# vedrocks15/Gradient-Based-Path-Tracing

Hardware: AMD Instinct MI355X
Metric: GDPT Msamples/s (base+4 offset) + Poisson ms, cbox 512x512 (higher is better)
Workload: dtype f64

## Files before the change

gradient-based-path-tracing_amd/csrc/hip/capi_device.hip:

```cpp
#include "../../../include/gdpt.h"
#include "../capi_common.h"
#include "../device_scene.h"
#include "../host/scene_prepare.h"
#include "poisson_kernels.h"
#include "recon_l1.h"
#include "recon_weighted.h"
#include "render_kernels.h"
#include "scene_internal.h"

#include <hip/hip_runtime.h>

#include <algorithm>
#include <cmath>
#include <cstdlib>
#include <cstring>
#include <exception>
#include <memory>
#include <string>
#include <thread>
#include <vector>

namespace {

using gdpt::ck;
// ... 178 lines not shown
            if (!capturing) join_scratch(sc);
            sc->need_fence = true;
        }
        ss.partials.alloc(need, "hipMalloc(work-item partials)");
    }
    if (!overlap) {
        if (!capturing) {
            sc->join();
            if (ss.used) ck(hipStreamWaitEvent(stream, ss.released, 0), "hipStreamWaitEvent(launch scratch)");
        }
    } else {
        if (sc->have_caller && stream != sc->last_caller) {
            for (auto &o : sc->scratch) ck(hipStreamWaitEvent(stream, o.rendered, 0), "hipStreamWaitEvent(render stream)");
            sc->need_fence = true;
        }
        if (sc->need_fence || !prev_entry) {
            for (auto &st : sc->render_stream) ck(hipStreamWaitEvent(st, entry, 0), "hipStreamWaitEvent(fence)");
            sc->need_fence = false;
        } else
            ck(hipStreamWaitEvent(sc->render_stream[k], prev_entry, 0), "hipStreamWaitEvent(previous call)");
        if (ss.used) ck(hipStreamWaitEvent(sc->render_stream[k], ss.released, 0), "hipStreamWaitEvent(launch scratch)");
    }
    sc->have_caller = true; sc->last_caller = stream;
    return ss;
}

gdpt::RenderLaunch begin_launch(GdptScene *sc, const Band &b, bool path, int take_pct, hipStream_t stream, const GdptRenderStats *stats, ScratchClaim *claim) {
    auto knob = [](const char *name, int def) { return gdpt::debug_knob_int(name, def); };
    const DevSceneView &v = sc->view;
    gdpt::RouteInputs in{};
    in.path = path; in.rng_scheme = b.rng; in.shift_mode = b.shift; in.max_depth = b.max_depth; in.rr_depth = v.rr_depth;
    in.one_sided = sc->traits.one_sided; in.has_rough = sc->traits.has_rough; in.lambert_only = sc->traits.lambert_only; in.material_mask = sc->traits.material_mask;
    in.has_spheres = v.num_spheres != 0; in.const_textures = v.all_textures_constant != 0; in.has_envmap = v.has_envmap != 0;
    in.fits_lds = gdpt::scene_fits_lds(v.num_nodes, v.num_prims, v.num_tris, v.num_materials, v.num_lights, sc->traits.bvh_depth);
    in.fits_lds_wide = gdpt::scene_fits_lds_wide(v.num_nodes4, v.num_prims, v.num_tris, v.num_materials, v.num_lights, sc->traits.wide_stack_need);
    in.force_eager = knob("force_eager", 0) != 0; in.no_lds_scene = knob("no_lds_scene", 0) != 0; in.lds_wide = knob("lds_wide", 1) != 0;
// ... 6 lines not shown
    rl.spp = b.spp; rl.stream_spp = b.stream_spp; rl.first_sample = b.first_sample; rl.row_begin = b.row_begin; rl.row_end = b.row_end; rl.max_depth = b.max_depth;
    rl.count_traversal = stats && stats->nodes_visited == ~0ull;
    rl.force_log2k = knob("log2k", -1);
    rl.thresh_a = knob("keep_frac", -1); rl.thresh_c = knob("search_frac", -1);
    rl.num_cus = sc->num_cus; rl.blocks_per_cu = knob("blocks_per_cu", 0);
    const bool capturing = is_capturing(stream);
    const bool overlap = !stats && gdpt::can_overlap(rl.route) && !capturing && knob("no_render_overlap", 0) == 0;
    size_t need = 0;
    if (gdpt::is_persistent(rl.route)) {
        rl.plan = gdpt::make_chunk_plan(b.spp, rl.force_log2k, (long long)v.cam.width * b.plan_rows, gdpt::resident_lanes(rl), take_pct);
        need = (size_t)16 * (size_t)gdpt::band_slots(v.cam.width, b.row_end - b.row_begin) * (size_t)rl.plan.n;
    }
    GdptLaunchScratch &ss = claim_scratch(sc, overlap, capturing, need, stream);
    rl.counters = ss.counters; sc->d_counters = ss.counters;
    if (gdpt::is_persistent(rl.route)) { rl.partials = ss.partials; rl.queue_head = ss.queue; }
    if (overlap) { rl.kernel_stream = sc->render_stream[sc->overlapped & 1]; rl.kernel_done = ss.rendered; }
    claim->set = &ss; claim->record_release = !capturing;
    return rl;
}

void run_launch(GdptScene *sc, const gdpt::RenderLaunch &rl, const ScratchClaim &claim, const Band &b, hipStream_t stream, GdptRenderStats *stats) {
    const bool stamped = gdpt::is_stamped(rl.route);
    const hipStream_t ks = rl.kernel_stream ? rl.kernel_stream : stream;
    if (rl.kernel_stream) sc->in_flight = true;
    ck(hipMemsetAsync(rl.counters, 0, sizeof(gdpt::RenderCounters), ks), "hipMemsetAsync(counters)");
    if (stamped) ck(hipMemsetAsync(&rl.counters->stamps[12], 0xFF, 2 * sizeof(unsigned long long), ks), "hipMemsetAsync(stamps)");
    if (stats) ck(hipEventRecord(sc->ev0, stream), "hipEventRecord");
    gdpt::launch_render(sc->view, rl, stream);
    if (rl.kernel_stream) sc->overlapped++;
    if (claim.record_release) { ck(hipEventRecord(claim.set->released, stream), "hipEventRecord(launch scratch)"); claim.set->used = true; }
    if (!stats) return;
    ck(hipEventRecord(sc->ev1, stream), "hipEventRecord");
    ck(hipMemcpyAsync(sc->h_counters, rl.counters, sizeof(gdpt::RenderCounters), hipMemcpyDeviceToHost, stream), "hipMemcpyAsync(counters)");
    ck(hipStreamSynchronize(stream), "hipStreamSynchronize(render)");
    float ms = 0;
    ck(hipEventElapsedTime(&ms, sc->ev0, sc->ev1), "hipEventElapsedTime");
    const gdpt::RenderCounters &c = *sc->h_counters;
    std::memset(stats, 0, sizeof(*stats));
    stats->samples = (uint64_t)sc->view.cam.width * (uint64_t)(b.row_end - b.row_begin) * (uint64_t)b.spp;
    stats->rays = c.rays; stats->bounces = c.bounces; stats->nonfinite_samples = c.nonfinite;
// ... 449 lines not shown
```

gradient-based-path-tracing_amd/csrc/hip/device_trace.h:

```cpp
#pragma once
#include "device_bsdf.h"

namespace gd {

struct Hit { float t, u, v, ngx, ngy, ngz; int gid; };

struct TraceCounters { unsigned nodes, prims, node_trips, leaf_trips, wave_steps, lane_steps; };
GD bool wave_leader() { return (int)(threadIdx.x & 63) == __ffsll((unsigned long long)__ballot(1)) - 1; }

GD bool tri_hit(const float o[3], const float d[3], float tnear, float tfar, const DevPrim &tr, float &t, float &u, float &v) {
#pragma clang fp contract(off)
    const float *e1 = tr.e1, *e2 = tr.e2;
    float px = d[1] * e2[2] - d[2] * e2[1];
    float py = d[2] * e2[0] - d[0] * e2[2];
    float pz = d[0] * e2[1] - d[1] * e2[0];
    float det = e1[0] * px + e1[1] * py + e1[2] * pz;
    if (!(det != 0.0f)) return false;
    float inv = 1.0f / det;
    float sx = o[0] - tr.v0[0], sy = o[1] - tr.v0[1], sz = o[2] - tr.v0[2];
    u = (sx * px + sy * py + sz * pz) * inv;
    if (!(u >= 0.0f && u <= 1.0f)) return false;
    float qx = sy * e1[2] - sz * e1[1];
    float qy = sz * e1[0] - sx * e1[2];
    float qz = sx * e1[1] - sy * e1[0];
// ... 170 lines not shown
GD D2 filter_sample(int type, double param, double rx, double ry) {
    D2 o;
    if (type == GDPT_FILTER_BOX) { o.x = (2 * rx - 1) * (param / 2); o.y = (2 * ry - 1) * (param / 2); }
    else if (type == GDPT_FILTER_GAUSSIAN) {
        double r = param * sqrt(-2 * log(fmax(rx, 1e-8)));
        double s, c;
        sincospi(2.0 * ry, &s, &c);
        o.x = r * c; o.y = r * s;
    } else {
        double h = param / 2;
        o.x = rx < 0.5 ? h * (sqrt(2 * rx) - 1) : h * (1 - sqrt(1 - 2 * (rx - 0.5)));
        o.y = ry < 0.5 ? h * (sqrt(2 * ry) - 1) : h * (1 - sqrt(1 - 2 * (ry - 0.5)));
    }
    return o;
}
GD D3 xform_point(const double *m, D3 p) {
    double tx = m[0] * p.x + m[1] * p.y + m[2] * p.z + m[3];
    double ty = m[4] * p.x + m[5] * p.y + m[6] * p.z + m[7];
    double tz = m[8] * p.x + m[9] * p.y + m[10] * p.z + m[11];
    double tw = m[12] * p.x + m[13] * p.y + m[14] * p.z + m[15];
    double inv_w = 1.0 / tw;
    return mk(tx * inv_w, ty * inv_w, tz * inv_w);
}
GD D3 xform_vector(const double *m, D3 v) {
    return mk(m[0] * v.x + m[1] * v.y + m[2] * v.z, m[4] * v.x + m[5] * v.y + m[6] * v.z, m[8] * v.x + m[9] * v.y + m[10] * v.z);
}
struct FilterCache { double dx, dy, ox, oy; };
template <bool PIXEL_SPACE = false>
GD Ray sample_primary(const DevCamera &cam, double sx, double sy, FilterCache *cache = nullptr, bool store = false) {
    const bool exact = PIXEL_SPACE && cam.pow2_film != 0;
    if (PIXEL_SPACE && !exact) { sx = sx / cam.width; sy = sy / cam.height; }
    double ppx = exact ? sx : sx * cam.width, ppy = exact ? sy : sy * cam.height;
    double fx = floor(ppx), fy = floor(ppy);
    D2 off;
    if (cache && !store && cache->dx == ppx - fx && cache->dy == ppy - fy) { off.x = cache->ox; off.y = cache->oy; }
    else {
        off = filter_sample(cam.filter_type, cam.filter_param, ppx - fx, ppy - fy);
        if (cache && store) { cache->dx = ppx - fx; cache->dy = ppy - fy; cache->ox = off.x; cache->oy = off.y; }
    }
    double rx, ry;
    if (exact) { rx = (fx + 0.5 + off.x) * cam.inv_width; ry = (fy + 0.5 + off.y) * cam.inv_height; }
    else { rx = (fx + 0.5 + off.x) / cam.width; ry = (fy + 0.5 + off.y) / cam.height; }
    D3 pt = xform_point(cam.sample_to_cam, mk(rx, ry, 0.0));
    D3 dir = normalize(pt);
    Ray r;
    r.org = mk(cam.org[0], cam.org[1], cam.org[2]);
    r.dir = normalize(xform_vector(cam.cam_to_world, dir));
    r.tnear = 0; r.tfar = __builtin_huge_val();
    return r;
}

}
```

gradient-based-path-tracing_amd/csrc/hip/render_device.h:

```cpp
#pragma once
#include "render_kernels.h"
#include "device_trace.h"
#include "../leaf_cursor.h"

namespace gd {

constexpr int kBlock = 256;
constexpr int kLdsSceneBytes = 20 * 1024;
constexpr int kLdsSceneLevels = 12;

struct LaneCounters { unsigned rays, bounces, nonfinite; };

enum { SEG_QUEUE = 0, SEG_TRACE = 1, SEG_VERTEX = 2, SEG_CONSUME = 3, SEG_BSDF = 4, SEG_FINISH = 5, SEG_CAMERA = 6, SEG_STEPS = 7, SEG_PUBLISH = 8, SEG_TAKE = 9, SEG_ITEM = 10, SEG_COUNT = 12, SEG_T_START = 12, SEG_T_DRY = 13, SEG_T_END = 14, SEG_SLOTS = 16 };
template <bool ON> struct Stamps {
    unsigned long long *slot;
    GD void start(unsigned long long *wave_row) {
        if (ON) { slot = wave_row; if ((threadIdx.x & 63) == 0) { for (int i = 0; i < SEG_COUNT; i++) slot[i] = 0; slot[SEG_COUNT] = __builtin_amdgcn_s_memtime(); } }
    }
    GD void mark(int seg) {
        if (ON) {
            __builtin_amdgcn_sched_barrier(0);
            const unsigned long long t = __builtin_amdgcn_s_memtime();
            __builtin_amdgcn_s_waitcnt(0xC07F);
            if ((int)(threadIdx.x & 63) == __ffsll((unsigned long long)__ballot(1)) - 1) { slot[seg] += t - slot[SEG_COUNT]; slot[SEG_COUNT] = t; }
// ... 556 lines not shown
            }
            if (!stop) {
                L.throughput = L.throughput * (G * f) / (p2 * rr_prob);
                L.num_vertices++;
                if (first) L.mats = (L.mats & 0xFFF) | ((nv.material_id & 0xFFF) << 12);
                if (!loop_allows(max_depth, L.num_vertices)) stop = true;
            }
        }
        if (!stop) act = ACT_BOUNCE;
        else if (first) { L.kc = C_AFTER_BOUNCE1 << 2; act = ACT_OFFSETS; }
        else { acc_no_offsets(acc, lp.radiance(), L.contrib, L.prob, spp, lc); act = ACT_NEXT_SAMPLE; }
    }
    stamps.mark(SEG_CONSUME);
    const bool off_valid = (st0 == S_OFFSET) && hit && nv.material_id == L.mat0();
    const bool off_resample = off_valid && (L.cmode() == C_AFTER_BOUNCE1 || L.cmode() == C_BROKE_BOUNCE2);
    bool sampled = false;
    BsdfSample bs; bs.dir_out = splat(0); bs.eta = 0; bs.roughness = 0;
    D3 f = splat(0);
    double pdf = 0;
    if (act == ACT_BOUNCE || off_resample) {
        D2 ruv; double rw;
        if (act == ACT_BOUNCE) {
            lc.bounces++;
            Pcg r; r.state = L.rng_state; r.inc = L.rng_inc;
            ruv.x = pcg_real(r); ruv.y = pcg_real(r); rw = pcg_real(r);
            L.rng_state = r.state;
            if (SERIAL_RNG && L.num_vertices == 3) { L.ruv1 = ruv; L.rw1 = rw; }
        } else if (SERIAL_RNG) { ruv = L.ruv1; rw = L.rw1; }
        else {
            Pcg r2 = pcg_init(base + (unsigned long long)L.s);
            (void)pcg_next(r2); (void)pcg_next(r2);
            ruv.x = pcg_real(r2); ruv.y = pcg_real(r2); rw = pcg_real(r2);
        }
        const D3 dir_view = -ray.dir;
// ... 15 lines not shown
            }
            if (alive) { cX = c0 * jac; wgt = L.prob / (L.prob + 1.0 * jac); }
        }
        bool flagged = (L.kc & kKcNonfinite) != 0;
        acc_offset(acc, k, L.contrib, cX, wgt, L.prob, spp, lc, flagged);
        if (flagged) L.kc |= kKcNonfinite;
        if (k == 3) { acc_base(acc, lp.radiance(), L.prob, spp, lc, flagged); L.kc &= ~kKcNonfinite; act = ACT_NEXT_SAMPLE; }
        else { L.kc = (L.kc & ~3) | (k + 1); act = ACT_OFFSET_RAY; }
    } else if (act == ACT_BOUNCE) {
        if (!sampled) act = ACT_NEXT_SAMPLE;
        else {
            if (pdf <= 0) {
                if (L.num_vertices == 3) { L.kc = C_BROKE_BOUNCE1 << 2; act = ACT_OFFSETS; }
                else if (L.num_vertices == 4 && L.mat0() == L.mat1()) { L.kc = C_BROKE_BOUNCE2 << 2; act = ACT_OFFSETS; }
                else { acc_no_offsets(acc, lp.radiance(), L.contrib, L.prob, spp, lc); act = ACT_NEXT_SAMPLE; }
            } else {
                L.org = nv.position; L.dir = bs.dir_out; L.f = f; L.pdf = pdf; L.st = S_BOUNCE;
            }
        }
    }
    stamps.mark(SEG_FINISH);
    if (act == ACT_OFFSETS) { L.kc &= ~3; act = ACT_OFFSET_RAY; }
    if (act == ACT_NEXT_SAMPLE) {
        L.s++;
        if (L.s >= L.s_end) L.st = S_DONE; else act = ACT_PRIMARY_RAY;
    }
    if (L.st == S_BOUNCE && act == ACT_BOUNCE) trav_init(sv, tv, __builtin_huge_val());
    return act;
}

template <bool SERIAL_RNG, class STAMPS = Stamps<false>>
GD void lane_camera(const DevSceneView &sv, int act, int x, int y, unsigned long long base, Lane &L, Trav &tv, LanePriv &lp, STAMPS *stp = nullptr) {
    STAMPS none{}; STAMPS &stamps = stp ? *stp : none;
    const DevCamera &cam = sv.cam;
    if (act == ACT_PRIMARY_RAY || act == ACT_OFFSET_RAY) {
        double rx, ry;
        int ox = 0, oy = 0;
        if (act == ACT_PRIMARY_RAY) {
            Pcg r;
            if (!SERIAL_RNG) r = pcg_init(base + (unsigned long long)L.s);
            else { r.state = L.rng_state; r.inc = L.rng_inc; }
            rx = pcg_real(r); ry = pcg_real(r);
            L.rng_state = r.state; L.rng_inc = r.inc;
            if (SERIAL_RNG) { L.rng_x = rx; L.rng_y = ry; }
            L.st = S_PRIMARY;
        } else {
            if (SERIAL_RNG) { rx = L.rng_x; ry = L.rng_y; }
            else { Pcg r2 = pcg_init(base + (unsigned long long)L.s); rx = pcg_real(r2); ry = pcg_real(r2); }
            const int k = L.k();
            ox = (k == 0) ? -1 : (k == 1 ? 1 : 0); oy = (k == 2) ? 1 : (k == 3 ? -1 : 0);
            L.st = S_OFFSET;
        }
        FilterCache fc;
        if (act == ACT_OFFSET_RAY) fc = lp.fc();
        Ray r = sample_primary<true>(cam, (x + ox) + rx, (y + oy) + ry, &fc, act == ACT_PRIMARY_RAY);
        if (act == ACT_PRIMARY_RAY) lp.set_fc(fc);
        L.org = r.org; L.dir = r.dir;
        trav_init(sv, tv, __builtin_huge_val());
    }
    stamps.mark(SEG_CAMERA);
}

template <bool LAMBERT, bool SERIAL_RNG, class ACC, class STAMPS = Stamps<false>, int PLAIN = 0>
GD void lane_step(const DevSceneView &sv, const TraceCtx &tx, int max_depth, double spp, int x, int y, unsigned long long base,
                  Lane &L, Trav &tv, LanePriv &lp, ACC &acc, LaneCounters &lc, TraceCounters &tc, STAMPS *stp = nullptr) {
    const int act = lane_consume<LAMBERT, SERIAL_RNG, ACC, STAMPS, PLAIN>(sv, tx, max_depth, spp, base, L, tv, lp, acc, lc, tc, stp);
    lane_camera<SERIAL_RNG, STAMPS>(sv, act, x, y, base, L, tv, lp, stp);
}

GD bool lane_tracing(int st) { return st == S_PRIMARY || st == S_BOUNCE || st == S_OFFSET; }
template <class TC>
GD void trace_pending(const DevSceneView &sv, const TraceCtx &tx, const Lane &L, Trav &tv, int keep_frac, int search_frac, TraceCounters &tc) {
    const bool pending = lane_tracing(L.st) && tv.cur != kTravDone;
    const unsigned long long m = __ballot(pending);
    if (m == 0ull) return;
    const int stop_below = (__popcll(m) * keep_frac) >> 8;
    if (pending) trav_run<TC>(sv, tx, L.org, L.dir, (L.st == S_BOUNCE) ? (float)sv.isect_eps : 0.0f, __builtin_huge_valf(), tv, stop_below, search_frac, tc);
}
GD bool lane_ready(const Lane &L, const Trav &tv) { return L.st == S_START || (lane_tracing(L.st) && tv.cur == kTravDone); }

GD unsigned wave_sum_u32(unsigned v) {
#pragma unroll
// ... 107 lines not shown
                next = (long long)got;
                end = min((long long)got + want, a.num_items);
                seen_head = end;
                if (next >= a.num_items) { exhausted = true; end = next; }
            }
            const int avail = (int)(end - next);
            const int rank = __popcll(m_idle & ((1ull << (tid & 63)) - 1ull));
            if (idle && rank < avail) item = next + rank;
            const int n_idle = __popcll(m_idle);
            next += (n_idle < avail) ? n_idle : avail;
        }
        return item;
    }
};

template <bool LAMBERT, bool LDS_SCENE, bool WIDE, bool WW, bool STAMPED = false, int PLAIN = 0, int LEAF_K = (LDS_SCENE && !GDPT_SPEC_LEAF ? GDPT_LDS_LEAF_K : 0)>
__global__ __launch_bounds__(kBlock, 2) void gdpt_render_phases(DevSceneView sv, KernelArgs a) {
    __shared__ int s_stack_fixed[LDS_SCENE ? kLdsSceneLevels * kBlock : 1];
    __shared__ __attribute__((aligned(16))) unsigned char s_scene[LDS_SCENE ? kLdsSceneBytes : 16];
    __shared__ double s_acc[15 * kBlock];
    __shared__ double s_priv[kPrivDoubles * kBlock];
    __shared__ int s_chunks[66];
    extern __shared__ __attribute__((aligned(16))) unsigned char s_dyn[];
    int *s_stack = LDS_SCENE ? s_stack_fixed : (int *)s_dyn;
    const int tid = threadIdx.x;
    if (tid <= a.num_chunks && tid < 66) s_chunks[tid] = a.chunk_begin[tid];
    TraceCtx tx = setup_trace<LDS_SCENE, WIDE>(sv, s_scene, s_stack, tid, kBlock, a.count != 0);
    if (!LDS_SCENE) __syncthreads();
    const int W = sv.cam.width;
    const double spp = (double)a.spp;
    AccLds acc; acc.slot = s_acc + tid; acc.stride = kBlock;
    acc.init();
    LanePriv lp; lp.slot = s_priv + tid; lp.stride = kBlock;
    LaneCounters lc = {0, 0, 0};
    TraceCounters tc = {0, 0, 0, 0, 0, 0};
    Lane L;
    Trav tv;
    trav_init(sv, tv, __builtin_huge_val());
    L.s = 0; L.s_end = 0; L.st = S_DONE;
    L.kc = 0; L.num_vertices = 0; L.mats = 0xFFFFFF; L.rng_state = 0; L.rng_inc = 1;
    L.org = L.dir = splat(0);
    int x = 0, y = 0;
    unsigned long long base = 0;
    long long my_item = -1;
    WaveQueue wq;
    __shared__ unsigned long long s_stamps[STAMPED ? (kBlock / 64) * (SEG_COUNT + 1) : 1];
    Stamps<STAMPED> stamps;
    stamps.start(s_stamps + (STAMPED ? (tid >> 6) * (SEG_COUNT + 1) : 0));
    unsigned long long t_dry = ~0ull;
    if (STAMPED && (tid & 63) == 0) atomicMin(&a.counters->stamps[SEG_T_START], __builtin_amdgcn_s_memrealtime());
    constexpr bool QUEUE_MID = LAMBERT;
    auto hand_out = [&](int &act) __attribute__((always_inline)) {
        const bool idle = (L.st == S_DONE);
        if (idle && my_item >= 0) {
            Accum r = acc.result();
            typedef double d2 __attribute__((ext_vector_type(2)));
            d2 *dst = (d2 *)(a.partials + (size_t)my_item * 16);
            dst[0] = d2{r.r.x, r.r.y}; dst[1] = d2{r.r.z, r.dx0.x}; dst[2] = d2{r.dx0.y, r.dx0.z}; dst[3] = d2{r.dy0.x, r.dy0.y};
            dst[4] = d2{r.dy0.z, r.dx1.x}; dst[5] = d2{r.dx1.y, r.dx1.z}; dst[6] = d2{r.dy1.x, r.dy1.y}; dst[7] = d2{r.dy1.z, 0.0};
            acc.init();
            my_item = -1;
        }
        stamps.mark(SEG_PUBLISH);
        const long long got_item = wq.take(a, idle, tid);
        stamps.mark(SEG_TAKE);
        if (STAMPED && wq.exhausted && t_dry == ~0ull) t_dry = __builtin_amdgcn_s_memrealtime();
        if (got_item >= 0) {
            my_item = got_item;
            int s0, s1;
            const bool inside = item_to_pixel(a, W, (unsigned)my_item, x, y, s0, s1, s_chunks);
            base = ((unsigned long long)y * W + x) * (unsigned long long)a.stream_spp;
            L.s = s0; L.s_end = s1;
            if (inside && s0 < s1) act = ACT_PRIMARY_RAY;
        }
        stamps.mark(SEG_ITEM);
    };
    for (;;) {
        int act = ACT_NONE;
        if (!QUEUE_MID) {
            hand_out(act);
            if (act == ACT_PRIMARY_RAY) L.st = S_START;
            if (!__any(L.st != S_DONE)) { if (wq.exhausted) break; else continue; }
            stamps.mark(SEG_QUEUE);
        }
        trace_pending<TraceCfg<WW, WIDE, !LDS_SCENE, !(PLAIN & kPlainNoSpheres), !LDS_SCENE, LEAF_K>>(sv, tx, L, tv, a.thresh_a, a.thresh_c, tc);
        stamps.mark(SEG_TRACE);
        stamps.tick(SEG_STEPS);
        act = ACT_NONE;
        if (lane_ready(L, tv)) {
            if (tx.count) { tc.lane_steps++; if (wave_leader()) tc.wave_steps++; }
            act = lane_consume<LAMBERT, false, AccLds, Stamps<STAMPED>, PLAIN>(sv, tx, a.max_depth, spp, base, L, tv, lp, acc, lc, tc, &stamps);
        }
        if (QUEUE_MID) hand_out(act);
        lane_camera<false, Stamps<STAMPED>>(sv, act, x, y, base, L, tv, lp, &stamps);
        if (QUEUE_MID) {
            if (!__any(L.st != S_DONE) && wq.exhausted) break;
            stamps.mark(SEG_QUEUE);
        }
    }
    flush_counters(a, lc, tc, a.count != 0);
    if (STAMPED && (tid & 63) == 0) {
        for (int i = 0; i < SEG_COUNT; i++) atomicAdd(&a.counters->stamps[i], stamps.get(i));
        atomicMin(&a.counters->stamps[SEG_T_DRY], t_dry);
        atomicMax(&a.counters->stamps[SEG_T_END], __builtin_amdgcn_s_memrealtime());
    }
}

#ifdef GDPT_BUILD_REDUCE
__global__ __launch_bounds__(256) void gdpt_reduce_partials(KernelArgs a, int W) {
// ... 246 lines not shown
```

gradient-based-path-tracing_amd/csrc/hip/render_kernels.h:

```cpp
#pragma once
#include "../device_scene.h"
#include <hip/hip_runtime.h>

namespace gdpt {

constexpr int kMaxChunks = 64;
struct ChunkPlan { int n; int begin[kMaxChunks + 1]; };

struct RenderCounters {
    unsigned long long rays, bounces, nonfinite, nodes, prims;
    unsigned long long wave_node_trips, wave_leaf_trips, wave_steps, lane_steps;
    unsigned long long stamps[16];
};

enum class Route : int {
    LAMBERT_PLAIN_LDS_CONST, LAMBERT_PLAIN_LDS_TEX, LAMBERT_PLAIN_HBM_CONST, LAMBERT_PLAIN_HBM_TEX,
    LAMBERT_LDS_WIDE, LAMBERT_LDS_BVH2, LAMBERT_HBM,
    LAMBERT_STAMPED_LDS_PLAIN, LAMBERT_STAMPED_LDS, LAMBERT_STAMPED_HBM,
    GENERAL_SET_A_DISNEY_DIFFUSE, GENERAL_SET_A_DISNEY_METAL, GENERAL_SET_B_DISNEY_CLEARCOAT, GENERAL_SET_B_DISNEY_SHEEN,
    GENERAL_LDS_WIDE, GENERAL_LDS_BVH2, GENERAL_HBM,
    TWOSIDED_LDS, TWOSIDED_HBM, TWOSIDED_HBM_GLASS,
    WAVEFRONT_LAMBERT, WAVEFRONT_GENERAL,
    EAGER, TILE_EAGER, TILE_PHASES_LAMBERT, TILE_PHASES_GENERAL,
    RECONNECT_LDS_LAMBERT, RECONNECT_HBM_LAMBERT, RECONNECT_GENERAL,
// ... 48 lines not shown
    unsigned long long *wf_state;
    unsigned *wf_live;
    void *wf_aux;
    int wf_sort;
    float wf_bounds[6];
    unsigned *wf_counters;
    unsigned *wf_host;
    hipEvent_t wf_event;
    int wf_slots;
    int replay_per_step;
    bool whole_leaf_trips;
    double *partials;
    unsigned long long *queue_head;
    hipStream_t kernel_stream;
    hipEvent_t kernel_done;
};
bool scene_fits_lds(int num_nodes, int num_prims, int num_tris, int num_materials, int num_lights, int bvh_depth);
bool scene_fits_lds_wide(int num_nodes4, int num_prims, int num_tris, int num_materials, int num_lights, int wide_stack_need);

inline long long resident_lanes(const RenderLaunch &rl) { return (long long)rl.num_cus * (rl.blocks_per_cu > 0 ? rl.blocks_per_cu : 2) * 256; }
inline long long band_slots(int width, int rows) { return (long long)((width + 15) / 16) * ((rows + 15) / 16) * 256; }
size_t twosided_log_bytes(unsigned blocks);
unsigned persistent_blocks(const RenderLaunch &rl, long long num_items);
ChunkPlan make_chunk_plan(int spp, int force_log2k, long long pixels, long long lanes, int take_pct = 0);

int wf_words();
int wf_max_generations();
int wf_slot_count(long long num_items);
size_t wf_aux_bytes(int slots);
void launch_render(const DevSceneView &sv, const RenderLaunch &rl, hipStream_t stream);
// ... 9 lines not shown
```

gradient-based-path-tracing_amd/csrc/hip/render_kernels.hip:

```cpp
#include "render_twosided.h"
#include "render_wavefront.h"

#include "../capi_common.h"
#include <stdexcept>
#include <string>

namespace gdpt {

namespace {
thread_local const char *g_route = "";
const char *const kRouteNames[] = {
    "lambert_plain/lds_const", "lambert_plain/lds_tex", "lambert_plain/hbm_const", "lambert_plain/hbm_tex",
    "lambert/lds_wide", "lambert/lds_bvh2", "lambert/hbm",
    "lambert_stamped/lds_plain", "lambert_stamped/lds", "lambert_stamped/hbm",
    "general_set_a/disney_diffuse", "general_set_a/disney_metal", "general_set_b/disney_clearcoat", "general_set_b/disney_sheen",
    "general/lds_wide", "general/lds_bvh2", "general/hbm",
    "twosided/lds", "twosided/hbm", "twosided/hbm_glass",
    "wavefront/lambert", "wavefront/general",
    "eager", "tile_eager", "tile_phases_lambert", "tile_phases_general",
    "reconnect/lds_lambert", "reconnect/hbm_lambert", "reconnect/general",
    "path/tile", "path/eager",
    "path_persistent/lds_lambert_plain", "path_persistent/lds_lambert", "path_persistent/lds_lambert_env",
    "path_persistent/hbm_lambert", "path_persistent/hbm_lambert_env",
    "path_persistent/lds_general", "path_persistent/lds_general_env", "path_persistent/hbm_general", "path_persistent/hbm_general_env",
// ... 70 lines not shown
    a.tile_w = ppb >= 16 ? 16 : ppb;
    a.tile_h = ppb / a.tile_w;
    a.tiles_x = (W + a.tile_w - 1) / a.tile_w;
    return dim3((unsigned)(a.tiles_x * ((rows + a.tile_h - 1) / a.tile_h)));
}

static dim3 start_queue(gd::KernelArgs &a, const RenderLaunch &rl, int W, hipStream_t stream) {
    a.num_chunks = rl.plan.n;
    for (int c = 0; c <= rl.plan.n; c++) a.chunk_begin[c] = rl.first_sample + rl.plan.begin[c];
    a.tiles_x = (W + 15) / 16;
    a.num_slots = band_slots(W, rl.row_end - rl.row_begin);
    a.num_items = a.num_slots * rl.plan.n;
    if (a.num_items >= (1LL << 32)) throw std::runtime_error("launch_render: image band too large for the 32-bit work queue");
    a.partials = rl.partials; a.queue_head = rl.queue_head;
    if (!a.partials || !a.queue_head) throw std::runtime_error("launch_render: work-queue buffers missing");
    if (hipMemsetAsync(a.queue_head, 0, sizeof(unsigned long long), stream) != hipSuccess) throw std::runtime_error("launch_render: queue reset failed");
    return dim3(persistent_blocks(rl, a.num_items));
}

int wf_words() { return gd::WF_WORDS; }
int wf_max_generations() { return gd::kWfMaxGen; }
int wf_slot_count(long long num_items) {
    long long n = num_items < (1LL << 21) ? num_items : (1LL << 21);
    n = (n + gd::kBlock - 1) / gd::kBlock * gd::kBlock;
    return (int)(n < gd::kBlock ? gd::kBlock : n);
}
namespace {
struct WfAux { size_t rays, hits, keys, hist, offsets, blocks, ovf, total; };
WfAux wf_aux_layout(int slots) {
    WfAux l{};
    size_t off = 0;
// ... 48 lines not shown
    for (;;) {
        ckh(hipMemcpyAsync(rl.wf_host, rl.wf_counters + 2 * gd::kWfMaxGen + (gen - 1), sizeof(unsigned), hipMemcpyDeviceToHost, stream), "hipMemcpyAsync(wavefront live count)");
        ckh(hipEventRecord(rl.wf_event, stream), "hipEventRecord");
        const bool room = gen + chunk <= gd::kWfMaxGen;
        if (room) enqueue_chunk();
        ckh(hipEventSynchronize(rl.wf_event), "hipEventSynchronize");
        if (*rl.wf_host == 0u) break;
        if (*rl.wf_host < active_bound) active_bound = *rl.wf_host;
        if (!room) throw std::runtime_error("launch_render: wavefront generation limit reached");
    }
}

void launch_render(const DevSceneView &sv, const RenderLaunch &rl, hipStream_t stream) {
    const Route r = rl.route;
    if (rl.kernel_stream && (!can_overlap(r) || !rl.kernel_done)) throw std::runtime_error("launch_render: this route does not overlap");
    const hipStream_t ks = rl.kernel_stream ? rl.kernel_stream : stream;
    gd::KernelArgs a{};
    a.spp = rl.spp; a.stream_spp = rl.stream_spp; a.first_sample = rl.first_sample; a.row_begin = rl.row_begin; a.row_end = rl.row_end; a.max_depth = rl.max_depth;
    a.img = rl.img; a.cx0 = rl.cx0; a.cy0 = rl.cy0; a.cx1 = rl.cx1; a.cy1 = rl.cy1; a.counters = rl.counters;
    a.thresh_a = rl.thresh_a >= 0 ? (rl.thresh_a > 255 ? 255 : rl.thresh_a) : 64;
    a.thresh_c = rl.thresh_c >= 0 ? (rl.thresh_c > 255 ? 255 : rl.thresh_c) : 112;
    a.count = rl.count_traversal ? 1 : 0;
    const int W = sv.cam.width, rows = rl.row_end - rl.row_begin;
    if (W <= 0 || rows <= 0 || rl.spp <= 0) throw std::runtime_error("launch_render: empty image band or spp <= 0");
    if (rl.first_sample < 0 || (long long)rl.first_sample + rl.spp > (long long)rl.stream_spp) throw std::runtime_error("launch_render: sample window outside its stream block");
    const int ntx = (W + 15) / 16, nty = (sv.cam.height + 15) / 16;
    dim3 grid((unsigned)((ntx * nty + 63) / 64));
    if (is_persistent(r)) {
        a.stack_levels = rl.wide_stack_need > 0 ? rl.wide_stack_need : GDPT_BVH_MAX_DEPTH;
        a.replay_per_step = rl.replay_per_step >= 1 ? rl.replay_per_step : 4;
// ... 143 lines not shown
```

Measured before the change: 2123.

## Enqueue resets early, read camera from kernarg, slice-based work queue

Counter and queue resets move into scratch claiming on the render stream, so they are ordered ahead of the cross-call fence and are not re-issued at launch. In the persistent render kernel, the wave work queue becomes a slice queue that sizes each atomic grab to the remaining work and decodes item coordinates incrementally. The camera is read directly from the kernarg segment through a constant address space pointer, and traversal init is split out of camera and consume into a separate arm step. These changes aim to cut register pressure, scalar loads and launch-side serialization, but they add reliance on the camera sitting at offset zero of the kernel arguments and more complex queue logic.

```diff
diff --git a/gradient-based-path-tracing_amd/csrc/hip/capi_device.hip b/gradient-based-path-tracing_amd/csrc/hip/capi_device.hip
--- a/gradient-based-path-tracing_amd/csrc/hip/capi_device.hip
+++ b/gradient-based-path-tracing_amd/csrc/hip/capi_device.hip
@@ -216,12 +216,15 @@
             for (auto &o : sc->scratch) ck(hipStreamWaitEvent(stream, o.rendered, 0), "hipStreamWaitEvent(render stream)");
             sc->need_fence = true;
         }
+        if (ss.used) ck(hipStreamWaitEvent(sc->render_stream[k], ss.released, 0), "hipStreamWaitEvent(launch scratch)");
+        sc->in_flight = true;
+        ck(hipMemsetAsync(ss.counters, 0, sizeof(gdpt::RenderCounters), sc->render_stream[k]), "hipMemsetAsync(counters)");
+        ck(hipMemsetAsync(ss.queue, 0, sizeof(unsigned long long), sc->render_stream[k]), "hipMemsetAsync(queue)");
         if (sc->need_fence || !prev_entry) {
             for (auto &st : sc->render_stream) ck(hipStreamWaitEvent(st, entry, 0), "hipStreamWaitEvent(fence)");
             sc->need_fence = false;
         } else
             ck(hipStreamWaitEvent(sc->render_stream[k], prev_entry, 0), "hipStreamWaitEvent(previous call)");
-        if (ss.used) ck(hipStreamWaitEvent(sc->render_stream[k], ss.released, 0), "hipStreamWaitEvent(launch scratch)");
     }
     sc->have_caller = true; sc->last_caller = stream;
     return ss;
@@ -258,7 +261,7 @@
     GdptLaunchScratch &ss = claim_scratch(sc, overlap, capturing, need, stream);
     rl.counters = ss.counters; sc->d_counters = ss.counters;
     if (gdpt::is_persistent(rl.route)) { rl.partials = ss.partials; rl.queue_head = ss.queue; }
-    if (overlap) { rl.kernel_stream = sc->render_stream[sc->overlapped & 1]; rl.kernel_done = ss.rendered; }
+    if (overlap) { rl.kernel_stream = sc->render_stream[sc->overlapped & 1]; rl.kernel_done = ss.rendered; rl.resets_enqueued = true; }
     claim->set = &ss; claim->record_release = !capturing;
     return rl;
 }
@@ -267,7 +270,7 @@
     const bool stamped = gdpt::is_stamped(rl.route);
     const hipStream_t ks = rl.kernel_stream ? rl.kernel_stream : stream;
     if (rl.kernel_stream) sc->in_flight = true;
-    ck(hipMemsetAsync(rl.counters, 0, sizeof(gdpt::RenderCounters), ks), "hipMemsetAsync(counters)");
+    if (!rl.resets_enqueued) ck(hipMemsetAsync(rl.counters, 0, sizeof(gdpt::RenderCounters), ks), "hipMemsetAsync(counters)");
     if (stamped) ck(hipMemsetAsync(&rl.counters->stamps[12], 0xFF, 2 * sizeof(unsigned long long), ks), "hipMemsetAsync(stamps)");
     if (stats) ck(hipEventRecord(sc->ev0, stream), "hipEventRecord");
     gdpt::launch_render(sc->view, rl, stream);
diff --git a/gradient-based-path-tracing_amd/csrc/hip/device_trace.h b/gradient-based-path-tracing_amd/csrc/hip/device_trace.h
--- a/gradient-based-path-tracing_amd/csrc/hip/device_trace.h
+++ b/gradient-based-path-tracing_amd/csrc/hip/device_trace.h
@@ -208,7 +208,8 @@
     }
     return o;
 }
-GD D3 xform_point(const double *m, D3 p) {
+template <class M>
+GD D3 xform_point(M m, D3 p) {
     double tx = m[0] * p.x + m[1] * p.y + m[2] * p.z + m[3];
     double ty = m[4] * p.x + m[5] * p.y + m[6] * p.z + m[7];
     double tz = m[8] * p.x + m[9] * p.y + m[10] * p.z + m[11];
@@ -216,12 +217,14 @@
     double inv_w = 1.0 / tw;
     return mk(tx * inv_w, ty * inv_w, tz * inv_w);
 }
-GD D3 xform_vector(const double *m, D3 v) {
+template <class M>
+GD D3 xform_vector(M m, D3 v) {
     return mk(m[0] * v.x + m[1] * v.y + m[2] * v.z, m[4] * v.x + m[5] * v.y + m[6] * v.z, m[8] * v.x + m[9] * v.y + m[10] * v.z);
 }
 struct FilterCache { double dx, dy, ox, oy; };
-template <bool PIXEL_SPACE = false>
-GD Ray sample_primary(const DevCamera &cam, double sx, double sy, FilterCache *cache = nullptr, bool store = false) {
+typedef const __attribute__((address_space(4))) DevCamera CamConst;
+template <bool PIXEL_SPACE = false, class CAM = const DevCamera>
+GD Ray sample_primary(CAM &cam, double sx, double sy, FilterCache *cache = nullptr, bool store = false) {
     const bool exact = PIXEL_SPACE && cam.pow2_film != 0;
     if (PIXEL_SPACE && !exact) { sx = sx / cam.width; sy = sy / cam.height; }
     double ppx = exact ? sx : sx * cam.width, ppy = exact ? sy : sy * cam.height;
@@ -235,11 +238,11 @@
     double rx, ry;
     if (exact) { rx = (fx + 0.5 + off.x) * cam.inv_width; ry = (fy + 0.5 + off.y) * cam.inv_height; }
     else { rx = (fx + 0.5 + off.x) / cam.width; ry = (fy + 0.5 + off.y) / cam.height; }
-    D3 pt = xform_point(cam.sample_to_cam, mk(rx, ry, 0.0));
+    D3 pt = xform_point(&cam.sample_to_cam[0], mk(rx, ry, 0.0));
     D3 dir = normalize(pt);
     Ray r;
     r.org = mk(cam.org[0], cam.org[1], cam.org[2]);
-    r.dir = normalize(xform_vector(cam.cam_to_world, dir));
+    r.dir = normalize(xform_vector(&cam.cam_to_world[0], dir));
     r.tnear = 0; r.tfar = __builtin_huge_val();
     return r;
 }
diff --git a/gradient-based-path-tracing_amd/csrc/hip/render_device.h b/gradient-based-path-tracing_amd/csrc/hip/render_device.h
--- a/gradient-based-path-tracing_amd/csrc/hip/render_device.h
+++ b/gradient-based-path-tracing_amd/csrc/hip/render_device.h
@@ -2,6 +2,7 @@
 #include "render_kernels.h"
 #include "device_trace.h"
 #include "../leaf_cursor.h"
+#include "../item_slice.h"
 
 namespace gd {
 
@@ -594,10 +595,9 @@
     stamps.mark(SEG_CONSUME);
     const bool off_valid = (st0 == S_OFFSET) && hit && nv.material_id == L.mat0();
     const bool off_resample = off_valid && (L.cmode() == C_AFTER_BOUNCE1 || L.cmode() == C_BROKE_BOUNCE2);
-    bool sampled = false;
-    BsdfSample bs; bs.dir_out = splat(0); bs.eta = 0; bs.roughness = 0;
-    D3 f = splat(0);
-    double pdf = 0;
+    bool sampled = false, arm = false;
+    BsdfSample bs; D3 f; double pdf;
+    if (!LAMBERT) { bs.dir_out = splat(0); bs.eta = 0; bs.roughness = 0; f = splat(0); pdf = 0; }
     if (act == ACT_BOUNCE || off_resample) {
         D2 ruv; double rw;
         if (act == ACT_BOUNCE) {
@@ -643,25 +643,26 @@
                 if (L.num_vertices == 3) { L.kc = C_BROKE_BOUNCE1 << 2; act = ACT_OFFSETS; }
                 else if (L.num_vertices == 4 && L.mat0() == L.mat1()) { L.kc = C_BROKE_BOUNCE2 << 2; act = ACT_OFFSETS; }
                 else { acc_no_offsets(acc, lp.radiance(), L.contrib, L.prob, spp, lc); act = ACT_NEXT_SAMPLE; }
-            } else {
-                L.org = nv.position; L.dir = bs.dir_out; L.f = f; L.pdf = pdf; L.st = S_BOUNCE;
-            }
+            } else arm = true;
         }
     }
     stamps.mark(SEG_FINISH);
+    if (arm) { L.org = nv.position; L.dir = bs.dir_out; L.f = f; L.pdf = pdf; L.st = S_BOUNCE; }
     if (act == ACT_OFFSETS) { L.kc &= ~3; act = ACT_OFFSET_RAY; }
     if (act == ACT_NEXT_SAMPLE) {
         L.s++;
         if (L.s >= L.s_end) L.st = S_DONE; else act = ACT_PRIMARY_RAY;
     }
-    if (L.st == S_BOUNCE && act == ACT_BOUNCE) trav_init(sv, tv, __builtin_huge_val());
     return act;
 }
 
-template <bool SERIAL_RNG, class STAMPS = Stamps<false>>
-GD void lane_camera(const DevSceneView &sv, int act, int x, int y, unsigned long long base, Lane &L, Trav &tv, LanePriv &lp, STAMPS *stp = nullptr) {
+GD void lane_arm(const DevSceneView &sv, int act, Trav &tv) {
+    if (act == ACT_BOUNCE || act == ACT_PRIMARY_RAY || act == ACT_OFFSET_RAY) trav_init(sv, tv, __builtin_huge_val());
+}
+
+template <bool SERIAL_RNG, class STAMPS = Stamps<false>, class CAM = const DevCamera>
+GD void lane_camera(const DevSceneView &sv, CAM &cam, int act, int x, int y, unsigned long long base, Lane &L, Trav &tv, LanePriv &lp, STAMPS *stp = nullptr) {
     STAMPS none{}; STAMPS &stamps = stp ? *stp : none;
-    const DevCamera &cam = sv.cam;
     if (act == ACT_PRIMARY_RAY || act == ACT_OFFSET_RAY) {
         double rx, ry;
         int ox = 0, oy = 0;
@@ -685,7 +686,6 @@
         Ray r = sample_primary<true>(cam, (x + ox) + rx, (y + oy) + ry, &fc, act == ACT_PRIMARY_RAY);
         if (act == ACT_PRIMARY_RAY) lp.set_fc(fc);
         L.org = r.org; L.dir = r.dir;
-        trav_init(sv, tv, __builtin_huge_val());
     }
     stamps.mark(SEG_CAMERA);
 }
@@ -694,7 +694,8 @@
 GD void lane_step(const DevSceneView &sv, const TraceCtx &tx, int max_depth, double spp, int x, int y, unsigned long long base,
                   Lane &L, Trav &tv, LanePriv &lp, ACC &acc, LaneCounters &lc, TraceCounters &tc, STAMPS *stp = nullptr) {
     const int act = lane_consume<LAMBERT, SERIAL_RNG, ACC, STAMPS, PLAIN>(sv, tx, max_depth, spp, base, L, tv, lp, acc, lc, tc, stp);
-    lane_camera<SERIAL_RNG, STAMPS>(sv, act, x, y, base, L, tv, lp, stp);
+    lane_camera<SERIAL_RNG, STAMPS>(sv, sv.cam, act, x, y, base, L, tv, lp, stp);
+    lane_arm(sv, act, tv);
 }
 
 GD bool lane_tracing(int st) { return st == S_PRIMARY || st == S_BOUNCE || st == S_OFFSET; }
@@ -832,6 +833,50 @@
     }
 };
 
+constexpr unsigned kNoItem = 0xFFFFFFFFu;
+struct SliceQueue {
+    unsigned next = 0, end = 0, start = 0;
+    ItemSlice slice = {0, 0, 0, 0};
+    bool exhausted = false;
+    GD unsigned take(const KernelArgs &a, bool idle, int tid, ItemParts &parts) {
+        unsigned item = kNoItem;
+        const unsigned long long m_idle = __ballot(idle);
+        if (m_idle) {
+            const unsigned num_items = (unsigned)a.num_items, num_slots = (unsigned)a.num_slots, tiles_x = (unsigned)a.tiles_x;
+            if (next >= end && !exhausted) {
+                const unsigned left = num_items - end;
+                const unsigned waves = gridDim.x * (unsigned)(kBlock / 64);
+                const unsigned n_idle_now = (unsigned)__popcll(m_idle);
+                unsigned want = 64;
+                if (left < waves * 64u) { want = left / (waves * 2u); want = want > 64u ? 64u : (want < n_idle_now ? n_idle_now : want); }
+                unsigned long long got = 0;
+                if ((tid & 63) == 0) got = atomicAdd(a.queue_head, (unsigned long long)want);
+                const unsigned got_lo = (unsigned)__builtin_amdgcn_readlane((int)(unsigned)got, 0);
+                const unsigned got_hi = (unsigned)__builtin_amdgcn_readlane((int)(unsigned)(got >> 32), 0);
+                if (got_hi != 0u || got_lo >= num_items) { exhausted = true; next = end = start = num_items; }
+                else {
+                    next = start = got_lo;
+                    end = (want < num_items - got_lo) ? got_lo + want : num_items;
+                    slice = item_slice_begin(start, num_slots, tiles_x);
+                }
+            }
+            const unsigned avail = end - next;
+            const unsigned rank = (unsigned)__popcll(m_idle & ((1ull << (tid & 63)) - 1ull));
+            if (idle && rank < avail) { item = next + rank; parts = item_slice_at(slice, item - start, num_slots, tiles_x); }
+            const unsigned n_idle = (unsigned)__popcll(m_idle);
+            next += (n_idle < avail) ? n_idle : avail;
+        }
+        return item;
+    }
+};
+
+static_assert(offsetof(DevSceneView, cam) == 0, "camera_here reads the camera at the start of the kernel's first argument");
+GD CamConst &camera_here() {
+    CamConst *p = (CamConst *)__builtin_amdgcn_kernarg_segment_ptr();
+    asm volatile("" : "+s"(p));
+    return *p;
+}
+
 template <bool LAMBERT, bool LDS_SCENE, bool WIDE, bool WW, bool STAMPED = false, int PLAIN = 0, int LEAF_K = (LDS_SCENE && !GDPT_SPEC_LEAF ? GDPT_LDS_LEAF_K : 0)>
 __global__ __launch_bounds__(kBlock, 2) void gdpt_render_phases(DevSceneView sv, KernelArgs a) {
     __shared__ int s_stack_fixed[LDS_SCENE ? kLdsSceneLevels * kBlock : 1];
@@ -860,8 +905,8 @@
     L.org = L.dir = splat(0);
     int x = 0, y = 0;
     unsigned long long base = 0;
-    long long my_item = -1;
-    WaveQueue wq;
+    unsigned my_item = kNoItem;
+    SliceQueue wq;
     __shared__ unsigned long long s_stamps[STAMPED ? (kBlock / 64) * (SEG_COUNT + 1) : 1];
     Stamps<STAMPED> stamps;
     stamps.start(s_stamps + (STAMPED ? (tid >> 6) * (SEG_COUNT + 1) : 0));
@@ -870,23 +915,25 @@
     constexpr bool QUEUE_MID = LAMBERT;
     auto hand_out = [&](int &act) __attribute__((always_inline)) {
         const bool idle = (L.st == S_DONE);
-        if (idle && my_item >= 0) {
+        if (idle && my_item != kNoItem) {
             Accum r = acc.result();
             typedef double d2 __attribute__((ext_vector_type(2)));
             d2 *dst = (d2 *)(a.partials + (size_t)my_item * 16);
             dst[0] = d2{r.r.x, r.r.y}; dst[1] = d2{r.r.z, r.dx0.x}; dst[2] = d2{r.dx0.y, r.dx0.z}; dst[3] = d2{r.dy0.x, r.dy0.y};
             dst[4] = d2{r.dy0.z, r.dx1.x}; dst[5] = d2{r.dx1.y, r.dx1.z}; dst[6] = d2{r.dy1.x, r.dy1.y}; dst[7] = d2{r.dy1.z, 0.0};
             acc.init();
-            my_item = -1;
+            my_item = kNoItem;
         }
         stamps.mark(SEG_PUBLISH);
-        const long long got_item = wq.take(a, idle, tid);
+        ItemParts parts;
+        const unsigned got_item = wq.take(a, idle, tid, parts);
         stamps.mark(SEG_TAKE);
         if (STAMPED && wq.exhausted && t_dry == ~0ull) t_dry = __builtin_amdgcn_s_memrealtime();
-        if (got_item >= 0) {
+        if (got_item != kNoItem) {
             my_item = got_item;
-            int s0, s1;
-            const bool inside = item_to_pixel(a, W, (unsigned)my_item, x, y, s0, s1, s_chunks);
+            x = (int)(parts.tx * 16u + (parts.pin & 15u)); y = a.row_begin + (int)(parts.ty * 16u + (parts.pin >> 4));
+            const int s0 = s_chunks[parts.c], s1 = s_chunks[parts.c + 1];
+            const bool inside = x < W && y < a.row_end;
             base = ((unsigned long long)y * W + x) * (unsigned long long)a.stream_spp;
             L.s = s0; L.s_end = s1;
             if (inside && s0 < s1) act = ACT_PRIMARY_RAY;
@@ -910,7 +957,8 @@
             act = lane_consume<LAMBERT, false, AccLds, Stamps<STAMPED>, PLAIN>(sv, tx, a.max_depth, spp, base, L, tv, lp, acc, lc, tc, &stamps);
         }
         if (QUEUE_MID) hand_out(act);
-        lane_camera<false, Stamps<STAMPED>>(sv, act, x, y, base, L, tv, lp, &stamps);
+        lane_camera<false, Stamps<STAMPED>>(sv, camera_here(), act, x, y, base, L, tv, lp, &stamps);
+        lane_arm(sv, act, tv);
         if (QUEUE_MID) {
             if (!__any(L.st != S_DONE) && wq.exhausted) break;
             stamps.mark(SEG_QUEUE);
diff --git a/gradient-based-path-tracing_amd/csrc/hip/render_kernels.h b/gradient-based-path-tracing_amd/csrc/hip/render_kernels.h
--- a/gradient-based-path-tracing_amd/csrc/hip/render_kernels.h
+++ b/gradient-based-path-tracing_amd/csrc/hip/render_kernels.h
@@ -86,6 +86,7 @@
     unsigned long long *queue_head;
     hipStream_t kernel_stream;
     hipEvent_t kernel_done;
+    bool resets_enqueued;
 };
 bool scene_fits_lds(int num_nodes, int num_prims, int num_tris, int num_materials, int num_lights, int bvh_depth);
 bool scene_fits_lds_wide(int num_nodes4, int num_prims, int num_tris, int num_materials, int num_lights, int wide_stack_need);
diff --git a/gradient-based-path-tracing_amd/csrc/hip/render_kernels.hip b/gradient-based-path-tracing_amd/csrc/hip/render_kernels.hip
--- a/gradient-based-path-tracing_amd/csrc/hip/render_kernels.hip
+++ b/gradient-based-path-tracing_amd/csrc/hip/render_kernels.hip
@@ -108,7 +108,7 @@
     if (a.num_items >= (1LL << 32)) throw std::runtime_error("launch_render: image band too large for the 32-bit work queue");
     a.partials = rl.partials; a.queue_head = rl.queue_head;
     if (!a.partials || !a.queue_head) throw std::runtime_error("launch_render: work-queue buffers missing");
-    if (hipMemsetAsync(a.queue_head, 0, sizeof(unsigned long long), stream) != hipSuccess) throw std::runtime_error("launch_render: queue reset failed");
+    if (!rl.resets_enqueued && hipMemsetAsync(a.queue_head, 0, sizeof(unsigned long long), stream) != hipSuccess) throw std::runtime_error("launch_render: queue reset failed");
     return dim3(persistent_blocks(rl, a.num_items));
 }
 
@@ -187,6 +187,7 @@
 void launch_render(const DevSceneView &sv, const RenderLaunch &rl, hipStream_t stream) {
     const Route r = rl.route;
     if (rl.kernel_stream && (!can_overlap(r) || !rl.kernel_done)) throw std::runtime_error("launch_render: this route does not overlap");
+    if (rl.resets_enqueued && !rl.kernel_stream) throw std::runtime_error("launch_render: resets enqueued ahead of a launch that does not overlap");
     const hipStream_t ks = rl.kernel_stream ? rl.kernel_stream : stream;
     gd::KernelArgs a{};
     a.spp = rl.spp; a.stream_spp = rl.stream_spp; a.first_sample = rl.first_sample; a.row_begin = rl.row_begin; a.row_end = rl.row_end; a.max_depth = rl.max_depth;
diff --git a/gradient-based-path-tracing_amd/csrc/item_slice.h b/gradient-based-path-tracing_amd/csrc/item_slice.h
--- /dev/null
+++ b/gradient-based-path-tracing_amd/csrc/item_slice.h
@@ -0,0 +1,46 @@
+#pragma once
+
+#if defined(__HIPCC__)
+#define GDPT_ITEM_HD __host__ __device__ inline
+#else
+#define GDPT_ITEM_HD inline
+#endif
+
+namespace gd {
+
+constexpr unsigned kItemSliceMax = 64;
+
+struct ItemParts { unsigned c, pin, tx, ty; };
+
+GDPT_ITEM_HD ItemParts item_divide(unsigned item, unsigned num_slots, unsigned tiles_x) {
+    ItemParts p;
+    p.c = item / num_slots;
+    const unsigned pt = item - p.c * num_slots;
+    const unsigned tile = pt >> 8;
+    p.pin = pt & 255u;
+    p.ty = tile / tiles_x; p.tx = tile - p.ty * tiles_x;
+    return p;
+}
+
+struct ItemSlice { unsigned c0, pt0, tx0, ty0; };
+
+GDPT_ITEM_HD ItemSlice item_slice_begin(unsigned start, unsigned num_slots, unsigned tiles_x) {
+    const ItemParts p = item_divide(start, num_slots, tiles_x);
+    ItemSlice s;
+    s.c0 = p.c; s.pt0 = start - p.c * num_slots; s.tx0 = p.tx; s.ty0 = p.ty;
+    return s;
+}
+
+GDPT_ITEM_HD ItemParts item_slice_at(const ItemSlice &s, unsigned d, unsigned num_slots, unsigned tiles_x) {
+    ItemParts p;
+    const unsigned pt = s.pt0 + d;
+    p.pin = pt & 255u;
+    if (pt >= num_slots) { p.c = s.c0 + 1; p.tx = 0; p.ty = 0; return p; }
+    p.c = s.c0;
+    const bool step = (pt >> 8) != (s.pt0 >> 8);
+    p.tx = s.tx0 + (step ? 1u : 0u); p.ty = s.ty0;
+    if (p.tx == tiles_x) { p.tx = 0; p.ty = s.ty0 + 1; }
+    return p;
+}
+
+}
diff --git a/profiles/isa_loop_counts.py b/profiles/isa_loop_counts.py
--- /dev/null
+++ b/profiles/isa_loop_counts.py
@@ -0,0 +1,207 @@
+#!/usr/bin/env python3
+import argparse
+import collections
+import os
+import re
+import subprocess
+import sys
+import tempfile
+
+HERE = os.path.dirname(os.path.abspath(__file__))
+CSRC = os.path.join(os.path.dirname(HERE), "gradient-based-path-tracing_amd", "csrc")
+DEFAULT_KERNEL = "gdpt_render_phasesILb1ELb1ELb1ELb1ELb0ELi3ELi2EE"
+
+
+def makefile_hipflags(csrc):
+    text = open(os.path.join(csrc, "Makefile")).read()
+    arch = os.environ.get("ARCH") or re.search(r"^ARCH \?= (\S+)", text, re.M).group(1)
+    flags = re.search(r"^HIPFLAGS = (.*)$", text, re.M).group(1).replace("$(ARCH)", arch)
+    hipcc = os.environ.get("HIPCC") or re.search(r"^HIPCC \?= (\S+)", text, re.M).group(1)
+    out, cur, quote = [], "", False
+    i = 0
+    while i < len(flags):
+        c = flags[i]
+        if c == "\\" and i + 1 < len(flags):
+            cur += flags[i + 1]; i += 2; continue
+        if c.isspace():
+            if cur:
+                out.append(cur); cur = ""
+        else:
+            cur += c
+        i += 1
+    if cur:
+        out.append(cur)
+    return hipcc, out
+
+
+def compile_asm(csrc, tu, out):
+    hipcc, flags = makefile_hipflags(csrc)
+    cmd = [hipcc] + flags + ["-S", "--cuda-device-only", "-gline-tables-only", tu, "-o", out]
+    subprocess.check_call(cmd, cwd=csrc)
+
+
+def find_line(csrc, spec):
+    name, *pats = spec.split(":")
+    path = None
+    for root, _, files in os.walk(csrc):
+        if os.path.basename(name) in files and "build" not in os.path.relpath(root, csrc).split(os.sep)[0]:
+            path = os.path.join(root, os.path.basename(name)); break
+    if path is None:
+        sys.exit(f"{name}: not found under {csrc}")
+    lines = open(path).read().splitlines()
+    found, start = [], 0
+    for p in pats:
+        rx = re.compile(p)
+        for n in range(start, len(lines)):
+            if rx.search(lines[n]):
+                found.append(n + 1); start = n + 1; break
+        else:
+            sys.exit(f"{spec}: no line matches {p!r}")
+    return os.path.basename(name), found
+
+
+def classify(op):
+    if op.startswith("v_"):
+        return "vector"
+    if op.startswith("s_"):
+        return "scalar"
+    if op.startswith("ds_"):
+        return "LDS"
+    if op.startswith(("global_", "flat_", "buffer_", "scratch_")):
+        return "memory"
+    return "other"
+
+
+def kernel_instructions(asm_path, kernel):
+    files = {}
+    body, inside, name = [], False, None
+    cur = ("", 0, ())
+    label = re.compile(r"^([A-Za-z_.$][\w.$]*):")
+    for raw in open(asm_path, errors="replace"):
+        line, _, comment = raw.partition(";")
+        s = line.strip()
+        if not s:
+            continue
+        m = re.match(r"\.file\s+(\d+)\s+(?:\"([^\"]*)\"\s+)?\"([^\"]*)\"", s)
+        if m:
+            files[int(m.group(1))] = os.path.basename(m.group(3)); continue
+        m = label.match(s)
+        if m and not inside:
+            if kernel in m.group(1) and not m.group(1).startswith("."):
+                inside, name = True, m.group(1)
+            continue
+        if not inside:
+            continue
+        if s.startswith(".Lfunc_end") or s.startswith(".section") or s.startswith(".size"):
+            break
+        m = re.match(r"\.loc\s+(\d+)\s+(\d+)", s)
+        if m:
+            chain = re.findall(r"([^\s\[\]@]+):(\d+):\d+", comment)
+            frames = tuple((os.path.basename(f), int(l)) for f, l in chain)
+            own = next(((os.path.basename(f), int(l)) for f, l in chain if not os.path.isabs(f)), None)
+            if own is None:
+                own = (files.get(int(m.group(1)), "?"), int(m.group(2)))
+            cur = (own[0], own[1], frames); continue
+        if label.match(s):
+            body.append(("", label.match(s).group(1), cur[0], cur[1], cur[2])); continue
+        if s.startswith("."):
+            continue
+        parts = s.split(None, 1)
+        body.append((parts[0], parts[1] if len(parts) > 1 else "", cur[0], cur[1], cur[2]))
+    if name is None:
+        sys.exit(f"no kernel whose name contains {kernel!r} in {asm_path}")
+    return name, body
+
+
+def main():
+    ap = argparse.ArgumentParser(description=__doc__, formatter_class=argparse.RawDescriptionHelpFormatter)
+    ap.add_argument("--csrc", default=CSRC)
+    ap.add_argument("--tu", default="hip/render_phases_lambert_plain.hip")
+    ap.add_argument("--kernel", default=DEFAULT_KERNEL)
+    ap.add_argument("--begin", default=r"render_device.h:GD TraceCtx setup_trace:__syncthreads\(\);")
+    ap.add_argument("--end", default=r"render_device.h:GD unsigned wave_sum_u32:GD void reduce_and_store")
+    ap.add_argument("--top", type=int, default=40)
+    ap.add_argument("--asm", default=None)
+    ap.add_argument("--keep", default=None, help="write the compiled assembly to this file")
+    a = ap.parse_args()
+
+    tmp = None
+    asm = a.asm
+    if asm is None:
+        tmp = tempfile.TemporaryDirectory()
+        asm = os.path.join(tmp.name, "tu.s")
+        if a.keep:
+            asm = os.path.abspath(a.keep)
+        compile_asm(a.csrc, a.tu, asm)
+    name, body = kernel_instructions(asm, a.kernel)
+    labels_at = {}
+    instrs = []
+    for x in body:
+        if x[0] == "":
+            labels_at[x[1]] = len(instrs)
+        else:
+            instrs.append(x)
+    body = instrs
+    bfile, blines = find_line(a.csrc, a.begin)
+    efile, elines = find_line(a.csrc, a.end)
+    bline = blines[-1]
+    e0, e1 = elines[0], elines[-1]
+
+    begin = max((i for i, x in enumerate(body) if (bfile, bline) in x[4] or (x[2], x[3]) == (bfile, bline)), default=None)
+    if begin is None:
+        sys.exit(f"no instruction of the kernel is attributed to {bfile}:{bline}")
+    end = next((i for i in range(begin + 1, len(body)) if body[i][2] == efile and e0 <= body[i][3] < e1), len(body))
+    head = None
+    for lab, pos in sorted(labels_at.items(), key=lambda kv: kv[1]):
+        if begin < pos < end and any(lab in re.split(r"[\s,]+", body[i][1]) for i in range(pos, end) if "branch" in body[i][0]):
+            head = pos; break
+    if head is None:
+        sys.exit("no backward branch in the region: not a loop")
+    once = body[begin + 1:head]
+    loop = body[head:end]
+
+    def totals(seq):
+        c = collections.Counter(classify(x[0]) for x in seq)
+        return c
+    print(f"kernel  {name}")
+    kt = totals(body)
+    print(f"whole kernel: {kt['vector']} vector / {kt['scalar']} scalar / {kt['LDS']} LDS / {kt['memory']} memory / {kt['other']} other")
+    ot, lt = totals(once), totals(loop)
+    print(f"region {bfile}:{bline} .. {efile}:{e0}: {ot['vector'] + lt['vector']} vector / {ot['scalar'] + lt['scalar']} scalar / {ot['LDS'] + lt['LDS']} LDS / "
+          f"{ot['memory'] + lt['memory']} memory")
+    om = sum(1 for x in once if x[0].startswith("v_mov_"))
+    print(f"  in front of the loop head, once per kernel: {ot['vector']} vector (of which {om} register moves) / {ot['scalar']} scalar / {ot['LDS']} LDS / {ot['memory']} memory")
+    print(f"loop: {lt['vector']} vector / {lt['scalar']} scalar / {lt['LDS']} LDS / {lt['memory']} memory / {lt['other']} other")
+    moves = [x for x in loop if x[0].startswith("v_mov_")]
+    lanes = [x for x in loop if x[0].startswith(("v_readlane", "v_writelane", "v_readfirstlane"))]
+    by_op = collections.Counter(x[0] for x in moves + lanes)
+    zero = sum(1 for op, args, *_ in moves if re.search(r",\s*0$", args))
+    noline = sum(1 for x in moves if x[3] == 0)
+    nv = max(1, lt["vector"])
+    print(f"  register moves: {len(moves)} ({100.0 * len(moves) / nv:.1f} % of vector; {noline} at line 0, {zero} write literal 0)")
+    print(f"  lane access (SGPR spill lanes and broadcasts): {len(lanes)}")
+    print("  " + ", ".join(f"{op} {n}" for op, n in sorted(by_op.items())))
+
+    per = collections.defaultdict(collections.Counter)
+    for op, _, f, l, _fr in loop:
+        c = classify(op)
+        per[(f, l)][c] += 1
+        if op.startswith("v_mov_"):
+            per[(f, l)]["mov"] += 1
+        if op.startswith(("v_readlane", "v_writelane", "v_readfirstlane")):
+            per[(f, l)]["lane"] += 1
+    per_file = collections.defaultdict(collections.Counter)
+    for (f, l), c in per.items():
+        per_file[f].update(c)
+    print("by file:        vector scalar    LDS memory  (moves, lane access)")
+    for f, c in sorted(per_file.items(), key=lambda kv: -kv[1]["vector"]):
+        print(f"  {f or '(none)':24s} {c['vector']:6d} {c['scalar']:6d} {c['LDS']:6d} {c['memory']:6d}  ({c['mov']}, {c['lane']})")
+    print(f"by line, top {a.top} by vector count:")
+    for (f, l), c in sorted(per.items(), key=lambda kv: (-kv[1]["vector"], kv[0]))[:a.top]:
+        print(f"  {(f or '(none)') + ':' + str(l):32s} {c['vector']:6d} {c['scalar']:6d} {c['LDS']:6d} {c['memory']:6d}  ({c['mov']}, {c['lane']})")
+    if tmp:
+        tmp.cleanup()
+
+
+if __name__ == "__main__":
+    main()
```

After: 2160 (median of 6 runs). 1.8% higher.
